# huggingface/transformers

Hardware: AMD Instinct MI355X
Metric: fwd+bwd tokens/sec (whole job), Llama-3-8B seq=4096 (higher is better)
Workload: dtype bf16; 1 GPU; llama3-8b: LlamaForCausalLM fwd+bwd incl. lm_head + causal-LM loss, random-init bf16 weights, per-GPU batch 8 x seq 4096; model=llama3-8b, global_batch=8, seq_len=4096, parallelism=dp1

## Files before the change

transformers_amd/csrc/attention.hip:

```cpp
#include "attention_common.h"

namespace tamd {

#include "attention_fwd_kernel.inc"

}

#include "attention_bwd.inc"

using namespace tamd;

namespace {

#ifdef TAMD_DIAG
unsigned long long* g_attn_trace = nullptr;
#endif

template <typename T, int D>
int attn_fwd_launch(const AttnArgs& a, bool causal, hipStream_t s) {
  const size_t smem = (size_t)4 * kKB * D * 2;
  dim3 grid((unsigned)(a.nqt * a.heads_q * a.batch)), block(kAttnThreads);
  const bool mask = a.key_valid != nullptr;
  const bool drop = a.drop_thr != 0;
#define TAMD_AF(C_, M_, D_) hipLaunchKernelGGL((attn_fwd_kernel<T, D, C_, M_, D_>), grid, block, smem, s, a)
  if (drop) {
    if (causal)
      TAMD_AF(true, true, true);
    else
      TAMD_AF(false, true, true);
  } else if (causal) {
    if (mask)
      TAMD_AF(true, true, false);
    else
      TAMD_AF(true, false, false);
  } else {
    if (mask)
      TAMD_AF(false, true, false);
    else
      TAMD_AF(false, false, false);
  }
#undef TAMD_AF
  return launch_status();
}

template <typename T, int D>
int attn_decode_launch(const AttnArgs& a, bool causal, hipStream_t s) {
  const size_t smem = (size_t)4 * kKB * D * 2;
  dim3 grid((unsigned)(a.nqt * a.heads_q * a.batch * a.kv_splits)), block(kAttnThreads);
#define TAMD_AD(C_, L_) hipLaunchKernelGGL((attn_fwd_kernel<T, D, C_, true, false, true, L_>), grid, block, smem, s, a)
  if (a.seq_k_dev != nullptr) {
    if (causal)
      TAMD_AD(true, true);
    else
      TAMD_AD(false, true);
  } else {
    if (causal)
      TAMD_AD(true, false);
    else
      TAMD_AD(false, false);
  }
#undef TAMD_AD
  const int rows = a.batch * a.seq_q * a.heads_q;
  hipLaunchKernelGGL((attn_combine_kernel<T, D>), dim3((unsigned)rows), dim3(256), 0, s, a);
  return launch_status();
}

int attn_check(const tamd_attn_params* p) {
  if (!p || !p->q || !p->k || !p->v || !p->o) return TAMD_E_NULL;
  if (p->head_dim != 64 && p->head_dim != 128) return TAMD_E_SHAPE;
  if (p->batch <= 0 || p->heads_q <= 0 || p->heads_kv <= 0 || p->seq_q <= 0 || p->seq_k <= 0) return TAMD_E_SHAPE;
  if (p->heads_q % p->heads_kv != 0) return TAMD_E_SHAPE;
  if (p->dtype != TAMD_BF16 && p->dtype != TAMD_F16) return TAMD_E_DTYPE;
  if (!(p->dropout_p >= 0.f && p->dropout_p < 1.f)) return TAMD_E_ARG;
  if (p->q_start != nullptr && (!p->causal || p->seq_q != p->seq_k)) return TAMD_E_ARG;
  const int64_t strides[] = {p->q_stride_b, p->q_stride_s, p->q_stride_h, p->k_stride_b, p->k_stride_s, p->k_stride_h,
                             p->v_stride_b, p->v_stride_s, p->v_stride_h, p->o_stride_b, p->o_stride_s, p->o_stride_h};
  for (int64_t st : strides)
    if (st % 8 != 0) return TAMD_E_ALIGN;
  const int64_t row_strides[] = {p->q_stride_s, p->k_stride_s, p->v_stride_s, p->o_stride_s};
  const int64_t row_counts[] = {p->seq_q, p->seq_k, p->seq_k, p->seq_q};
  for (int i = 0; i < 4; ++i)
    if (row_counts[i] > 1 && (row_strides[i] < p->head_dim || row_strides[i] > ((int64_t)1 << 24))) return TAMD_E_ARG;
  if (!aligned16(p->q) || !aligned16(p->k) || !aligned16(p->v) || !aligned16(p->o)) return TAMD_E_ALIGN;
  return TAMD_OK;
}

AttnArgs make_args(const tamd_attn_params* p) {
  AttnArgs a;
  a.q = p->q;
  a.k = p->k;
  a.v = p->v;
  a.o = p->o;
// ... 159 lines not shown
```

transformers_amd/csrc/attention_bwd.inc:

```

namespace tamd {

#include "attention_bwd_dq_kernel.inc"

template <typename T, int D>
static int attn_bwd_launch(const AttnArgs& a, const tamd_attn_bwd_params* p, bool causal, hipStream_t s) {
  AttnBwdArgs g;
  g.f = a;
  g.dout = p->dout;
  g.dq = p->dq;
  g.dk = p->dk;
  g.dv = p->dv;
  g.delta = p->delta;
  g.scale = p->fwd.scale;
  g.rope_cos = p->rope_cos;
  g.rope_sin = p->rope_sin;
  g.rope_cos_batch = (int)p->rope_cos_batch;
  const bool mask = a.key_valid != nullptr;
  const bool drop = a.drop_thr != 0;
  {
    const size_t smem = (size_t)4 * kKB * D * 2;
    dim3 grid((unsigned)(a.nqt * a.heads_q * a.batch)), block(kAttnThreads);
#define TAMD_DQ(C_, M_, D_) hipLaunchKernelGGL((attn_bwd_dq_kernel<T, D, C_, M_, D_>), grid, block, smem, s, g)
    if (drop) {
      if (causal)
        TAMD_DQ(true, true, true);
      else
        TAMD_DQ(false, true, true);
    } else if (causal) {
      if (mask)
        TAMD_DQ(true, true, false);
      else
        TAMD_DQ(true, false, false);
    } else {
      if (mask)
        TAMD_DQ(false, true, false);
      else
        TAMD_DQ(false, false, false);
    }
#undef TAMD_DQ
  }
  const int st = launch_status();
  return st != 0 ? st : attn_bwd_dkdv_launch(g, __is_same(T, bf16_t) ? TAMD_BF16 : TAMD_F16, D, causal, s);
}

}
```

transformers_amd/csrc/attention_bwd_dq_kernel.inc:

```
template <typename T, int D, bool CAUSAL, bool HAS_MASK, bool DROP>
__global__ __launch_bounds__(kAttnThreads, 2) void attn_bwd_dq_kernel(AttnBwdArgs g) {
  const AttnArgs& a = g.f;
  constexpr int ROWB = D * 2, TILEB = kKB * ROWB, KS = D / 16, DT = D / 32, OROWB = ROWB + 16;
  TAMD_DYN_SMEM(smem);
  const int tid = threadIdx.x, lane = tid & 63;
  const int wave = wave_id_uniform();
  const int hi = lane >> 5, l31 = lane & 31;
  const int group = a.heads_q / a.heads_kv;
  int b, h, qt;
  {
    const int bid = blockIdx.x;
    const int per_grp = a.nqt * group;
    int gi, within;
    if (a.xcd_map) {
      const int xcd = bid & 7, j = bid >> 3;
      gi = (j / per_grp) * 8 + xcd;
      within = j % per_grp;
    } else {
      gi = bid / per_grp;
      within = bid % per_grp;
    }
    b = gi / a.heads_kv;
    h = (gi % a.heads_kv) * group + within % group;
    qt = a.nqt - 1 - within / group;
  }
  const int hkv = h / group;
  const int q0 = qt * kQB, qw0 = q0 + wave * 32, qrow = qw0 + l31;
  const int off = a.seq_k - a.seq_q;
  const T* Q = reinterpret_cast<const T*>(a.q) + (int64_t)b * a.qsb + (int64_t)h * a.qsh;
  const T* K = reinterpret_cast<const T*>(a.k) + (int64_t)b * a.ksb + (int64_t)hkv * a.ksh;
  const T* V = reinterpret_cast<const T*>(a.v) + (int64_t)b * a.vsb + (int64_t)hkv * a.vsh;
  const T* dO = reinterpret_cast<const T*>(g.dout) + (int64_t)b * a.osb + (int64_t)h * a.osh;

  const T* O = reinterpret_cast<const T*>(a.o) + (int64_t)b * a.osb + (int64_t)h * a.osh;
  u32x4 qf[KS], dof[KS];
  float dlt = 0.f;
#pragma unroll
  for (int ks = 0; ks < KS; ++ks) {
    const bool ok = qrow < a.seq_q;
    qf[ks] = ok ? ld16(Q + (int64_t)qrow * a.qss + ks * 16 + hi * 8) : u32x4{0, 0, 0, 0};
    dof[ks] = ok ? ld16(dO + (int64_t)qrow * a.oss + ks * 16 + hi * 8) : u32x4{0, 0, 0, 0};
    const u32x4 of = ok ? ld16(O + (int64_t)qrow * a.oss + ks * 16 + hi * 8) : u32x4{0, 0, 0, 0};
    float x[8], y[8];
    unpack16<T>(of, x);
    unpack16<T>(dof[ks], y);
#pragma unroll
    for (int e = 0; e < 8; ++e) dlt += x[e] * y[e];
  }
  dlt += swap32_f32(dlt);
#pragma unroll
  for (int ks = 0; ks < KS; ++ks) qf[ks] = scale_frag<T>(qf[ks], a.scale_log2, !a.q_prescaled);
  const int64_t stat_idx = ((int64_t)b * a.heads_q + h) * a.seq_q + qrow;
  const float nlse2 = (qrow < a.seq_q) ? -a.lse[stat_idx] * 1.44269504088896340736f : -INFINITY;
  constexpr bool S_FROM_LSE = !(HAS_MASK && D > 64);
  const f32x16 s_start = splat16(S_FROM_LSE ? nlse2 : 0.f);
  constexpr bool FOLD_DELTA = !DROP && !(HAS_MASK && D > 64);
  const f32x16 dp_start = splat16(FOLD_DELTA ? -dlt : 0.f);
  if (hi == 0 && qrow < a.seq_q) {
    g.delta[stat_idx] = -dlt;
    g.delta[(int64_t)a.batch * a.heads_q * a.seq_q + stat_idx] = nlse2;
  }
  const AttnDrop drop = attn_drop_ctx(a);
  const unsigned long long drop_base = drop.row_base((unsigned long long)b * a.heads_q + h, (qrow >> 1) <= ((a.seq_q - 1) >> 1) ? qrow : 0);
  const unsigned drop_lsh = (qrow & 1) ? 0u : 16u;

  const int klo = packed_klo(a, b, qrow);
  const int klo_max = (int)wave_max((float)klo), klo_min = -(int)wave_max(-(float)klo);

  TileOffsets<D> toff;
  toff.init(lane);
  const unsigned lds0 = lds_base_u32(smem);
  f32x16 dqacc[DT];
#pragma unroll
  for (int dt = 0; dt < DT; ++dt)
#pragma unroll
    for (int r = 0; r < 16; ++r) dqacc[dt][r] = 0.f;

  int kend = a.seq_k;
  if (CAUSAL) {
    const int lim = q0 + kQB + off;
    kend = lim < kend ? lim : kend;
    if (kend < 0) kend = 0;
  }
  const int nkt = (kend + kKB - 1) / kKB;
  TileFeed<D> feed, feedv;
  feed.init(a.kss, wave, lane);
  feedv.init(a.vss, wave, lane);
  static_assert(KS == 2 * TileFeed<D>::NI, "one piece per k-step of the first sub-tile");
  auto issue_piece = [&](int t, int rows, int buf, int n) {
    constexpr int NI = TileFeed<D>::NI;
    const unsigned k_off = (unsigned)buf * 2u * TILEB, v_off = k_off + TILEB;
    if (n < NI)
      feed.issue_one_rng(K + (int64_t)t * kKB * a.kss, rows, a.kss, smem, k_off, wave, n);
    else
      feedv.issue_one_rng(V + (int64_t)t * kKB * a.vss, rows, a.vss, smem, v_off, wave, n - NI);
  };
  auto tile_rows = [&](int t) { return a.seq_k - t * kKB < kKB ? a.seq_k - t * kKB : kKB; };
  auto issue = [&](int t, int rows, int buf) {
#pragma unroll
    for (int n = 0; n < KS; ++n) issue_piece(t, rows, buf, n);
  };
  const int t0 = (q0 < a.seq_q ? packed_klo(a, b, q0) : 0) / kKB;
  if (nkt > t0) issue(t0, tile_rows(t0), t0 & 1);
  wait_vmcnt0();
  block_sync();
  for (int t = t0; t < nkt; ++t) {
    const int cur = t & 1;
    const int tn = t + 1, rows_n = t + 1 < nkt ? tile_rows(t + 1) : 0;
    const unsigned k_off = (unsigned)cur * 2u * TILEB, v_off = k_off + TILEB;
    const int kt0 = t * kKB;
    const bool wave_active = (!CAUSAL || (kt0 <= qw0 + 31 + off)) && (kt0 + kKB > klo_min);
    if (!wave_active) issue(tn, rows_n, cur ^ 1);
    if (wave_active) {
      unsigned long long vmask = ~0ull;
      if (HAS_MASK) {
        const int kp = kt0 + lane;
        vmask = ballot64(kp < a.seq_k && (a.key_valid == nullptr || a.key_valid[(int64_t)b * a.seq_k + kp] != 0));
      }
      const bool need_mask = (HAS_MASK && vmask != ~0ull) || (kt0 + kKB > a.seq_k) || (CAUSAL && (kt0 + kKB - 1 > qw0 + off)) ||
                             (kt0 < klo_max);
      const unsigned kb = lds0 + k_off;
      u32x4 dsf[4];
      constexpr int NV = DT * 4;
      constexpr int VA = (DROP || (HAS_MASK && D > 64)) ? 2 : (NV < 4 ? NV : 4);
      u32x4 vr[VA + 1];
      auto creq = [&](int i) -> u32x4 {
        const int dt = i % DT, j = i / DT;
        const int rb = ((j >> 1) * 32 + (j & 1) * 16) * ROWB;
        const u32x2 lo = lds_read8_tr16_abs(kb + toff.tr[dt][0], rb);
        const u32x2 h2 = lds_read8_tr16_abs(kb + toff.tr[dt][1], rb);
        return u32x4{lo[0], lo[1], h2[0], h2[1]};
      };
      {
        constexpr int NA = 4 * KS;
        constexpr int KA = (DROP || (HAS_MASK && D > 64)) ? 2 : 3;
        u32x4 fr[KA + 1];
        auto areq = [&](int i) -> u32x4 {
          const int sub = i / (2 * KS), ks = (i >> 1) % KS;
          return lds_read16_abs(kb + toff.row[ks], sub * 32 * ROWB + (i & 1) * TILEB);
        };
#pragma unroll
        for (int i = 0; i < KA; ++i) fr[i] = areq(i);
#pragma unroll
        for (int sub = 0; sub < 2; ++sub) {
          f32x16 s, dp;
          if (S_FROM_LSE) {
            s = s_start;
          } else {
#pragma unroll
            for (int r = 0; r < 16; ++r) s[r] = 0.f;
          }
          if (FOLD_DELTA) {
            dp = dp_start;
          } else {
#pragma unroll
            for (int r = 0; r < 16; ++r) dp[r] = 0.f;
          }
#pragma unroll
          for (int k2 = 0; k2 < 2 * KS; ++k2) {
            const int i = sub * 2 * KS + k2;
            if (i + KA < NA) fr[(i + KA) % (KA + 1)] = areq(i + KA);
            if (KA >= 3) {
              if (!(i & 1)) constexpr_wait_frag2<KA - 1>(NA - 2 - i, fr[i % (KA + 1)], fr[(i + 1) % (KA + 1)]);
            } else {
              constexpr_wait_frag<KA>(NA - 1 - i, fr[i % (KA + 1)]);
            }
            if (k2 & 1)
              dp = mfma32<T>(fr[i % (KA + 1)], dof[k2 >> 1], dp);
            else
              s = mfma32<T>(fr[i % (KA + 1)], qf[k2 >> 1], s);
            if (sub == 0 && (k2 & 1)) issue_piece(tn, rows_n, cur ^ 1, k2 >> 1);
          }
          if (need_mask) {
#pragma unroll
            for (int r = 0; r < 16; ++r) {
              const int kl = sub * 32 + (r & 3) + 8 * (r >> 2) + 4 * hi;
              const int kp = kt0 + kl;
              bool vis = kp < a.seq_k && kp >= klo;
              if (CAUSAL) vis = vis && (kp <= qrow + off);
              if (HAS_MASK) vis = vis && ((vmask >> kl) & 1ull);
              s[r] = vis ? s[r] : -INFINITY;
            }
          }
          float ds[16];
          if (DROP) {
#pragma unroll
            for (int r = 0; r < 16; r += 4) {
              unsigned w0, w1;
              drop.words(drop_base + (unsigned long long)(((kt0 + sub * 32 + (r & 3) + 8 * (r >> 2) + 4 * hi) >> 1) + (qrow & 1)), w0, w1);
              dp[r] = drop.kept(pair_even_u32(w0), drop_lsh) ? dp[r] : 0.f;
              dp[r + 1] = drop.kept(pair_even_u32(w1), drop_lsh) ? dp[r + 1] : 0.f;
              dp[r + 2] = drop.kept(pair_odd_u32(w0), drop_lsh) ? dp[r + 2] : 0.f;
              dp[r + 3] = drop.kept(pair_odd_u32(w1), drop_lsh) ? dp[r + 3] : 0.f;
            }
          }
#pragma unroll
          for (int r = 0; r < 16; ++r)
            ds[r] = fast_exp2(S_FROM_LSE ? s[r] : s[r] + nlse2) * (DROP ? fmaf(dp[r], drop.scale, -dlt) : (FOLD_DELTA ? dp[r] : dp[r] - dlt));
          pack_c_to_b<T>(ds, &dsf[sub * 2]);
          pin_frags(dsf[sub * 2], dsf[sub * 2 + 1]);
            }
      }
      {
#pragma unroll
        for (int i = 0; i < VA; ++i) vr[i] = creq(i);
#pragma unroll
        for (int i = 0; i < NV; ++i) {
          if (i + VA < NV) vr[(i + VA) % (VA + 1)] = creq(i + VA);
          if (VA >= 3) {
            if (!(i & 1)) constexpr_wait_frag2<2 * (VA - 1)>(2 * (NV - 2 - i), vr[i % (VA + 1)], vr[(i + 1) % (VA + 1)]);
          } else {
            constexpr_wait_frag<2 * VA>(2 * (NV - 1 - i), vr[i % (VA + 1)]);
          }
          dqacc[i % DT] = mfma32<T>(vr[i % (VA + 1)], dsf[i / DT], dqacc[i % DT]);
        }
      }
    }
    wait_vmcnt0();
    block_sync();
  }
  T* dQ = reinterpret_cast<T*>(g.dq) + (int64_t)b * a.qsb + (int64_t)h * a.qsh;
  const int64_t crow0 = (g.rope_cos_batch == 1 ? 0 : (int64_t)b * a.seq_q) + qw0;
  store_rows_via_lds<T, D>(dqacc, g.scale, smem, (unsigned)wave * (32u * OROWB), dQ, a.qss, qw0, a.seq_q, lane,
                           reinterpret_cast<const T*>(g.rope_cos), reinterpret_cast<const T*>(g.rope_sin), crow0);
}
```

transformers_amd/csrc/attention_common.h:

```cpp
#pragma once
#include <stdlib.h>

#include "common.h"
#include "dropout.h"

namespace tamd {

template <int N>
struct IntC {
  static constexpr int value = N;
};

constexpr int kAttnThreads = 256;
constexpr int kQB = 128;
constexpr int kKB = 64;

__device__ __attribute__((aligned(16))) static const unsigned int g_zero16a[4] = {0u, 0u, 0u, 0u};

struct AttnArgs {
  const void* q;
  const void* k;
  const void* v;
  void* o;
  float* lse;
  const uint8_t* key_valid;
  const int* q_start;
  int batch, heads_q, heads_kv, seq_q, seq_k;
  int64_t qsb, qss, qsh, ksb, kss, ksh, vsb, vss, vsh, osb, oss, osh;
  float scale_log2;
  unsigned drop_thr;
  float drop_scale;
  unsigned seed_lo, seed_hi;
  const unsigned long long* seed_dev;
  int nqt;
  int xcd_map;
  int q_prescaled;
  unsigned long long* trace;
  float* o_part;
  float* lse_part;
  int kv_splits, tiles_per_split;
  const int* seq_k_dev;
};

#ifdef TAMD_DIAG
#define TAMD_ATTN_PHASE(i_)                              \
  if (tr) {                                              \
    asm volatile("" ::: "memory");                       \
    const unsigned long long now_ = device_clock();      \
    asm volatile("" ::: "memory");                       \
    ph[i_] += now_ - tlast;                              \
    tlast = now_;                                        \
  }
#else
#define TAMD_ATTN_PHASE(i_)
#endif

__device__ __forceinline__ AttnDrop attn_drop_ctx(const AttnArgs& a) {
  unsigned s0 = a.seed_lo, s1 = a.seed_hi;
  if (a.seed_dev != nullptr) {
    const unsigned long long mixed = attn_seed_mix(*a.seed_dev);
    s0 = (unsigned)mixed;
    s1 = (unsigned)(mixed >> 32);
  }
  return AttnDrop{a.drop_thr << 16, s0, s1, a.drop_scale, ((unsigned long long)a.seq_q + 1) >> 1,
                  ((unsigned long long)a.seq_k + 1) >> 1};
}

template <int D>
__device__ __forceinline__ int row_swz(int row) {
  return D == 128 ? (((row & 3) << 2) | ((row >> 2) & 3)) : ((((row >> 1) & 1) << 2) | ((row >> 2) & 3));
}

template <typename T, int D>
__device__ __forceinline__ void issue_kv_tile(const T* __restrict__ base, int64_t stride, int key0, int nkeys,
                                              char* smem, unsigned tile_off, int wave, int lane) {
  constexpr int ROWB = D * 2;
  constexpr int SLOTS = ROWB / 16;
  constexpr int RPI = 1024 / ROWB;
  constexpr int NI = (kKB * ROWB) / 1024 / 4;
#pragma unroll
  for (int i = 0; i < NI; ++i) {
    const int inst = wave * NI + i;
    const int r = inst * RPI + lane / SLOTS;
    const int p = lane % SLOTS;
    const int s = p ^ row_swz<D>(r);
    const int key = key0 + r;
    const void* src = (key < nkeys) ? (const void*)(base + (int64_t)key * stride + s * 8) : (const void*)g_zero16a;
    glds16(src, smem, tile_off + (unsigned)inst * 1024u);
  }
}

template <int D>
struct TileFeed {
  static constexpr int NI = (kKB * D * 2) / 1024 / 4;
  unsigned voff[NI];
  __device__ __forceinline__ void init(int64_t stride, int wave, int lane) {
    constexpr int ROWB = D * 2, SLOTS = ROWB / 16, RPI = 1024 / ROWB;
#pragma unroll
    for (int i = 0; i < NI; ++i) {
      const int inst = wave * NI + i;
      const int r = inst * RPI + lane / SLOTS;
      const int s = (lane % SLOTS) ^ row_swz<D>(r);
      voff[i] = (unsigned)(((int64_t)r * stride + s * 8) * 2);
    }
  }
  static __host__ __device__ __forceinline__ bool usable(int64_t stride) { return stride > 0 && stride * (kKB * 2) < ((int64_t)1 << 31); }
  template <typename T>
  __device__ __forceinline__ void issue_one(const T* __restrict__ first_row, char* smem, unsigned tile_off, int wave,
                                            int i) const {
    glds16_buf<0>(first_row, voff[i], smem, tile_off + (unsigned)(wave * NI + i) * 1024u);
  }
  template <typename T>
  __device__ __forceinline__ void issue_one_rng(const T* __restrict__ first_row, int rows, int64_t stride, char* smem,
                                                unsigned tile_off, int wave, int i) const {
    glds16_buf_rng(first_row, (unsigned)rows * (unsigned)stride * 2u, voff[i], smem, tile_off + (unsigned)(wave * NI + i) * 1024u);
  }
  template <typename T>
  __device__ __forceinline__ void issue(const T* __restrict__ first_row, char* smem, unsigned tile_off, int wave) const {
#pragma unroll
    for (int i = 0; i < NI; ++i) issue_one(first_row, smem, tile_off, wave, i);
  }
};

template <int D>
struct TileOffsets {
  unsigned row[D / 16];
  unsigned tr[D / 32][2];
  __device__ __forceinline__ void init(int lane) {
    constexpr int ROWB = D * 2;
    const int hi = lane >> 5, l31 = lane & 31, kq = (lane & 15) >> 2;
#pragma unroll
    for (int ks = 0; ks < D / 16; ++ks)
      row[ks] = (unsigned)l31 * ROWB + (unsigned)(((ks * 2 + hi) ^ row_swz<D>(l31)) * 16);
#pragma unroll
    for (int dt = 0; dt < D / 32; ++dt) {
      const int col = dt * 32 + 16 * ((lane >> 4) & 1) + 4 * (lane & 3);
#pragma unroll
      for (int t2 = 0; t2 < 2; ++t2) {
        const int r = 4 * hi + kq + 8 * t2;
        tr[dt][t2] = (unsigned)r * ROWB + (unsigned)(((col >> 3) ^ row_swz<D>(r)) * 16) + (unsigned)(col & 7) * 2u;
      }
    }
  }
  __device__ __forceinline__ u32x4 read_tr(const char* smem, unsigned tile_off, int dt, int j) const {
    const unsigned rb = (unsigned)(((j >> 1) * 32 + (j & 1) * 16) * (D * 2));
    const u32x2 lo = lds_read8_tr16(smem, tile_off + tr[dt][0] + rb);
    const u32x2 h2 = lds_read8_tr16(smem, tile_off + tr[dt][1] + rb);
    return u32x4{lo[0], lo[1], h2[0], h2[1]};
  }
  __device__ __forceinline__ u32x4 read_row(const char* smem, unsigned tile_off, int sub, int ks) const {
    return lds_read16(smem, tile_off + row[ks] + (unsigned)(sub * 32 * D * 2));
  }
};

template <int N>
__device__ __forceinline__ void wait_frag(u32x4& f) {
#if defined(__HIP_DEVICE_COMPILE__)
  asm volatile("s_waitcnt lgkmcnt(%1)" : "+v"(f) : "n"(N) : "memory");
#else
  (void)f;
#endif
}
__device__ __forceinline__ void pin_frags(u32x4& f0, u32x4& f1) {
#if defined(__HIP_DEVICE_COMPILE__)
  asm volatile("" : "+v"(f0), "+v"(f1));
#else
  (void)f0;
  (void)f1;
// ... 142 lines not shown
```

transformers_amd/csrc/attention_fwd_kernel.inc:

```
template <typename T, int D, bool CAUSAL, bool HAS_MASK, bool DROP, bool SPLIT = false, bool DEVLEN = false>
__global__ __launch_bounds__(kAttnThreads, (DROP && D > 64) ? 1 : ((D == 64 && !HAS_MASK && !DROP) ? 3 : 2)) void attn_fwd_kernel(AttnArgs a) {
  constexpr int ROWB = D * 2;
  constexpr int TILEB = kKB * ROWB;
  constexpr int KS = D / 16;
  constexpr int DT = D / 32;
  constexpr int OROWB = ROWB + 16;
  TAMD_DYN_SMEM(smem);
  const int tid = threadIdx.x, lane = tid & 63;
  const int wave = wave_id_uniform();
  const int hi = lane >> 5, l31 = lane & 31;

  const int group = a.heads_q / a.heads_kv;
  int b, h, qt;
  const int split = SPLIT ? (int)(blockIdx.x % (unsigned)a.kv_splits) : 0;
  {
    const int bid = SPLIT ? (int)(blockIdx.x / (unsigned)a.kv_splits) : (int)blockIdx.x;
    const int per_grp = a.nqt * group;
    int g, within;
    if (a.xcd_map) {
      const int xcd = bid & 7, j = bid >> 3;
      g = (j / per_grp) * 8 + xcd;
      within = j % per_grp;
    } else {
      g = bid / per_grp;
      within = bid % per_grp;
    }
    b = g / a.heads_kv;
    const int hkv = g % a.heads_kv;
    h = hkv * group + within % group;
    qt = a.nqt - 1 - within / group;
  }
  const int hkv = h / group;
  const int q0 = qt * kQB;
  static_assert(!DEVLEN || SPLIT, "key counts in device memory: the split-KV instantiations only");
  int seq_k = a.seq_k;
  if constexpr (SPLIT && DEVLEN) {
    int n = wave_uniform_i32(a.seq_k_dev[b]);
    n = n < a.seq_k ? n : a.seq_k;
    seq_k = n > 0 ? n : 0;
  }
  const int off = seq_k - a.seq_q;
  const T* Q = reinterpret_cast<const T*>(a.q) + (int64_t)b * a.qsb + (int64_t)h * a.qsh;
  const T* K = reinterpret_cast<const T*>(a.k) + (int64_t)b * a.ksb + (int64_t)hkv * a.ksh;
  const T* V = reinterpret_cast<const T*>(a.v) + (int64_t)b * a.vsb + (int64_t)hkv * a.vsh;

  const int qw0 = q0 + wave * 32;
  const int qrow = qw0 + l31;
  u32x4 qf[KS];
#pragma unroll
  for (int ks = 0; ks < KS; ++ks)
    qf[ks] = (qrow < a.seq_q) ? ld16(Q + (int64_t)qrow * a.qss + ks * 16 + hi * 8) : u32x4{0, 0, 0, 0};
#pragma unroll
  for (int ks = 0; ks < KS; ++ks) qf[ks] = scale_frag<T>(qf[ks], a.scale_log2, !a.q_prescaled);

  const int klo = packed_klo(a, b, qrow);
  const int klo_max = (int)wave_max((float)klo), klo_min = -(int)wave_max(-(float)klo);

  f32x16 oacc[DT];
#pragma unroll
  for (int dt = 0; dt < DT; ++dt)
#pragma unroll
    for (int r = 0; r < 16; ++r) oacc[dt][r] = 0.f;
  float m_run = -INFINITY, l_run = 0.f;
  f32x16 neg_m = splat16(0.f);

  int kend = seq_k;
  if (CAUSAL) {
    const int lim = q0 + kQB - 1 + off + 1;
    kend = lim < kend ? lim : kend;
    if (kend < 0) kend = 0;
  }
  const int nkt = (kend + kKB - 1) / kKB;

  TileOffsets<D> toff;
  toff.init(lane);
  const unsigned lds0 = lds_base_u32(smem);
  const AttnDrop drop = attn_drop_ctx(a);
  const unsigned long long drop_base = drop.row_base((unsigned long long)b * a.heads_q + h, (qrow >> 1) <= ((a.seq_q - 1) >> 1) ? qrow : 0);
  const unsigned drop_lsh = (qrow & 1) ? 0u : 16u;
  constexpr float kDeferThr = 6.f;

  TileFeed<D> feed, feedv;
  feed.init(a.kss, wave, lane);
  feedv.init(a.vss, wave, lane);
  auto issue_piece = [&](int t, int rows, int buf, int n) {
    constexpr int NI = TileFeed<D>::NI;
    const unsigned k_off = (unsigned)buf * 2u * TILEB, v_off = k_off + TILEB;
    if (n < NI)
      feed.issue_one_rng(K + (int64_t)t * kKB * a.kss, rows, a.kss, smem, k_off, wave, n);
    else
      feedv.issue_one_rng(V + (int64_t)t * kKB * a.vss, rows, a.vss, smem, v_off, wave, n - NI);
  };
  auto tile_rows = [&](int t) { return seq_k - t * kKB < kKB ? seq_k - t * kKB : kKB; };
  auto issue = [&](int t, int rows, int buf) {
#pragma unroll
    for (int n = 0; n < 2 * TileFeed<D>::NI; ++n) issue_piece(t, rows, buf, n);
  };
  const int t0f = (q0 < a.seq_q ? packed_klo(a, b, q0) : 0) / kKB;
  const int t0 = SPLIT ? (t0f > split * a.tiles_per_split ? t0f : split * a.tiles_per_split) : t0f;
  const int nkt_w = SPLIT ? (nkt < (split + 1) * a.tiles_per_split ? nkt : (split + 1) * a.tiles_per_split) : nkt;
  if (nkt_w > t0) issue(t0, tile_rows(t0), t0 & 1);
  wait_vmcnt0();
  block_sync();

#ifdef TAMD_DIAG
  const bool tr = a.trace != nullptr && blockIdx.x == 0;
  unsigned long long ph[8] = {0, 0, 0, 0, 0, 0, 0, 0}, tlast = tr ? device_clock() : 0ull;
#endif
  for (int t = t0; t < nkt_w; ++t) {
    const int cur = t & 1;
    const int tn = t + 1, rows_n = t + 1 < nkt_w ? tile_rows(t + 1) : 0;
    TAMD_ATTN_PHASE(0)
    const unsigned k_off = (unsigned)cur * 2u * TILEB, v_off = k_off + TILEB;
    const int kt0 = t * kKB;
    const bool wave_active = (!CAUSAL || (kt0 <= qw0 + 31 + off)) && (kt0 + kKB > klo_min);
    if (wave_active) {
      const unsigned kb = lds0 + k_off, vb = lds0 + v_off;
      f32x16 s[2] = {neg_m, neg_m};
      {
        constexpr int NM = 2 * KS;
        constexpr int KA = (DROP || (HAS_MASK && D > 64)) ? 2 : (NM < 8 ? NM : 8);
        u32x4 kr[KA + 1];
#pragma unroll
        for (int i = 0; i < KA; ++i) kr[i] = lds_read16_abs(kb + toff.row[i >> 1], (i & 1) * 32 * ROWB);
#pragma unroll
        for (int i = 0; i < NM; ++i) {
          if (i + KA < NM) kr[(i + KA) % (KA + 1)] = lds_read16_abs(kb + toff.row[(i + KA) >> 1], ((i + KA) & 1) * 32 * ROWB);
          if (KA >= 3) {
            if (!(i & 1)) constexpr_wait_frag2<KA - 1>(NM - 2 - i, kr[i % (KA + 1)], kr[(i + 1) % (KA + 1)]);
          } else {
            constexpr_wait_frag<KA>(NM - 1 - i, kr[i % (KA + 1)]);
          }
          s[i & 1] = mfma32<T>(kr[i % (KA + 1)], qf[i >> 1], s[i & 1]);
          if ((i & 1) && (i >> 1) < 2 * TileFeed<D>::NI) issue_piece(tn, rows_n, cur ^ 1, i >> 1);
        }
      }
      TAMD_ATTN_PHASE(1)
      constexpr int NV = DT * 4;
      constexpr int VA = (DROP || (HAS_MASK && D > 64)) ? 2 : (NV < 7 ? NV : 7);
      u32x4 vr[VA + 1];
      auto vreq = [&](int i) -> u32x4 {
        const int dt = i % DT, j = i / DT;
        const int rb = ((j >> 1) * 32 + (j & 1) * 16) * ROWB;
        const u32x2 lo = lds_read8_tr16_abs(vb + toff.tr[dt][0], rb);
        const u32x2 h2 = lds_read8_tr16_abs(vb + toff.tr[dt][1], rb);
        return u32x4{lo[0], lo[1], h2[0], h2[1]};
      };
#pragma unroll
      for (int i = 0; i < VA; ++i) vr[i] = vreq(i);
      unsigned long long vmask = ~0ull;
      if (HAS_MASK) {
        const int kp = kt0 + lane;
        vmask = ballot64(kp < seq_k && (a.key_valid == nullptr || a.key_valid[(int64_t)b * a.seq_k + kp] != 0));
      }
      const bool need_mask = (HAS_MASK && vmask != ~0ull) || (kt0 + kKB > seq_k) || (CAUSAL && (kt0 + kKB - 1 > qw0 + off)) ||
                             (kt0 < klo_max);
      if (need_mask) {
#pragma unroll
        for (int sub = 0; sub < 2; ++sub)
#pragma unroll
          for (int r = 0; r < 16; ++r) {
            const int kl = sub * 32 + (r & 3) + 8 * (r >> 2) + 4 * hi;
            const int kp = kt0 + kl;
            bool vis = kp < seq_k && kp >= klo;
            if (CAUSAL) vis = vis && (kp <= qrow + off);
            if (HAS_MASK) vis = vis && ((vmask >> kl) & 1ull);
            s[sub][r] = vis ? s[sub][r] : -INFINITY;
          }
      }
      float mx = s[0][0];
#pragma unroll
      for (int sub = 0; sub < 2; ++sub)
#pragma unroll
        for (int r = 0; r < 16; ++r) mx = fmaxf(mx, s[sub][r]);
      mx = fmaxf(mx, swap32_f32(mx));
      const float m_old = (m_run == -INFINITY) ? 0.f : m_run;
      const float m_tile = mx + m_old;
      if (ballot64(m_tile - m_run > kDeferThr) != 0ull) {
        const float m_new = fmaxf(m_run, m_tile);
        const float alpha = (m_new == -INFINITY) ? 1.f : fast_exp2(m_run - m_new);
        m_run = m_new;
        l_run *= alpha;
#pragma unroll
        for (int dt = 0; dt < DT; ++dt)
#pragma unroll
          for (int r = 0; r < 16; ++r) oacc[dt][r] *= alpha;
        const float m_ref = (m_new == -INFINITY) ? 0.f : m_new;
        const float shift = m_ref - m_old;
#pragma unroll
        for (int sub = 0; sub < 2; ++sub)
#pragma unroll
          for (int r = 0; r < 16; ++r) s[sub][r] -= shift;
        neg_m = splat16(-m_ref);
      }
      float psum = 0.f;
      u32x4 pf[4];
#pragma unroll
      for (int sub = 0; sub < 2; ++sub) {
        float p[16];
#pragma unroll
        for (int r = 0; r < 16; ++r) {
          p[r] = fast_exp2(s[sub][r]);
          psum += p[r];
        }
        if (DROP) {
#pragma unroll
          for (int r = 0; r < 16; r += 4) {
            unsigned w0, w1;
            drop.words(drop_base + (unsigned long long)(((kt0 + sub * 32 + (r & 3) + 8 * (r >> 2) + 4 * hi) >> 1) + (qrow & 1)), w0, w1);
            p[r] = drop.kept(pair_even_u32(w0), drop_lsh) ? p[r] : 0.f;
            p[r + 1] = drop.kept(pair_even_u32(w1), drop_lsh) ? p[r + 1] : 0.f;
            p[r + 2] = drop.kept(pair_odd_u32(w0), drop_lsh) ? p[r + 2] : 0.f;
            p[r + 3] = drop.kept(pair_odd_u32(w1), drop_lsh) ? p[r + 3] : 0.f;
          }
        }
#pragma unroll
        for (int st = 0; st < 2; ++st)
          pf[sub * 2 + st] = u32x4{pack2<T>(p[8 * st + 0], p[8 * st + 1]), pack2<T>(p[8 * st + 2], p[8 * st + 3]),
                                   pack2<T>(p[8 * st + 4], p[8 * st + 5]), pack2<T>(p[8 * st + 6], p[8 * st + 7])};
      }
      l_run += psum;
      TAMD_ATTN_PHASE(2)
#pragma unroll
      for (int i = 0; i < NV; ++i) {
        if (i + VA < NV) vr[(i + VA) % (VA + 1)] = vreq(i + VA);
        if (VA >= 3) {
          if (!(i & 1)) constexpr_wait_frag2<2 * (VA - 1)>(2 * (NV - 2 - i), vr[i % (VA + 1)], vr[(i + 1) % (VA + 1)]);
        } else {
          constexpr_wait_frag<2 * VA>(2 * (NV - 1 - i), vr[i % (VA + 1)]);
        }
        oacc[i % DT] = mfma32<T>(vr[i % (VA + 1)], pf[i / DT], oacc[i % DT]);
      }
      TAMD_ATTN_PHASE(3)
    } else {
      issue(tn, rows_n, cur ^ 1);
    }
    wait_vmcnt0();
    TAMD_ATTN_PHASE(4)
    block_sync();
    TAMD_ATTN_PHASE(5)
  }
#ifdef TAMD_DIAG
  if (tr && lane == 0) {
#pragma unroll
    for (int i = 0; i < 8; ++i) a.trace[wave * 8 + i] = ph[i];
  }
#endif

  l_run += swap32_f32(l_run);
  const float inv_l = (l_run > 0.f) ? (DROP ? drop.scale : 1.f) / l_run : 0.f;
  if (SPLIT) {
    if (qrow < a.seq_q) {
      const int64_t prow = (((int64_t)split * a.batch + b) * a.seq_q + qrow) * a.heads_q + h;
      if (hi == 0)
        a.lse_part[(((int64_t)split * a.batch + b) * a.heads_q + h) * a.seq_q + qrow] =
            (l_run > 0.f) ? (m_run + fast_log2(l_run)) * 0.69314718055994530942f : -INFINITY;
      float* dst = a.o_part + prow * D;
#pragma unroll
      for (int dt = 0; dt < DT; ++dt)
#pragma unroll
        for (int qd = 0; qd < 4; ++qd)
          st16(dst + dt * 32 + 8 * qd + 4 * hi,
               u32x4{f32_as_u32(oacc[dt][qd * 4 + 0] * inv_l), f32_as_u32(oacc[dt][qd * 4 + 1] * inv_l),
                     f32_as_u32(oacc[dt][qd * 4 + 2] * inv_l), f32_as_u32(oacc[dt][qd * 4 + 3] * inv_l)});
    }
    return;
  }
  if (a.lse != nullptr && hi == 0 && qrow < a.seq_q) {
    const float lse = (l_run > 0.f) ? (m_run + fast_log2(l_run)) * 0.69314718055994530942f : INFINITY;
    a.lse[((int64_t)b * a.heads_q + h) * a.seq_q + qrow] = lse;
  }
  const unsigned st_off = (unsigned)wave * (32u * OROWB);
#pragma unroll
  for (int dt = 0; dt < DT; ++dt)
#pragma unroll
    for (int qd = 0; qd < 4; ++qd) {
      const int d0 = dt * 32 + 8 * qd + 4 * hi;
      const u32x2 pk = {pack2<T>(oacc[dt][qd * 4 + 0] * inv_l, oacc[dt][qd * 4 + 1] * inv_l),
                        pack2<T>(oacc[dt][qd * 4 + 2] * inv_l, oacc[dt][qd * 4 + 3] * inv_l)};
      lds_write8(smem, st_off + (unsigned)l31 * OROWB + (unsigned)d0 * 2u, pk);
    }
  wave_lockstep_point();
  T* O = reinterpret_cast<T*>(a.o) + (int64_t)b * a.osb + (int64_t)h * a.osh;
  constexpr int SLOTS = ROWB / 16;
  constexpr int RPI = 64 / SLOTS;
#pragma unroll
  for (int it = 0; it < 32 / RPI; ++it) {
    const int row = it * RPI + lane / SLOTS, slot = lane % SLOTS;
    const int qr = qw0 + row;
    const u32x4 v = lds_read16(smem, st_off + (unsigned)row * OROWB + (unsigned)slot * 16u);
    if (qr < a.seq_q) st16(O + (int64_t)qr * a.oss + slot * 8, v);
  }
}

template <typename T, int D>
__global__ __launch_bounds__(256) void attn_combine_kernel(AttnArgs a) {
  __shared__ float part[4][D];
  __shared__ float wpart[4];
  const int wave = wave_id_uniform(), lane = threadIdx.x & 63;
  const int row = (int)blockIdx.x;
  const int h = row % a.heads_q, qrow = (row / a.heads_q) % a.seq_q, b = row / (a.heads_q * a.seq_q);
  const int64_t lse_stride = (int64_t)a.batch * a.heads_q * a.seq_q;
  const float* lse0 = a.lse_part + ((int64_t)b * a.heads_q + h) * a.seq_q + qrow;
  float mx = -INFINITY;
  for (int s = lane; s < a.kv_splits; s += 64) mx = fmaxf(mx, lse0[(int64_t)s * lse_stride]);
  mx = wave_max(mx);
  constexpr int PER = D / 64;
  float acc[PER], wsum = 0.f;
#pragma unroll
  for (int e = 0; e < PER; ++e) acc[e] = 0.f;
  const int64_t o_stride = (int64_t)a.batch * a.seq_q * a.heads_q * D;
  const float* o0 = a.o_part + (((int64_t)b * a.seq_q + qrow) * a.heads_q + h) * D + lane * PER;
#pragma unroll 4
  for (int s = wave; s < a.kv_splits; s += 4) {
    const float ls = lse0[(int64_t)s * lse_stride];
    const float w = (ls == -INFINITY) ? 0.f : __expf(ls - mx);
    wsum += w;
    const float* src = o0 + (int64_t)s * o_stride;
#pragma unroll
    for (int e = 0; e < PER; ++e) acc[e] += w * src[e];
  }
#pragma unroll
  for (int e = 0; e < PER; ++e) part[wave][lane * PER + e] = acc[e];
  if (lane == 0) wpart[wave] = wsum;
  block_sync();
  if (wave != 0) return;
  wsum = ((wpart[0] + wpart[1]) + wpart[2]) + wpart[3];
  const float inv = wsum > 0.f ? 1.f / wsum : 0.f;
  T* O = reinterpret_cast<T*>(a.o) + (int64_t)b * a.osb + (int64_t)qrow * a.oss + (int64_t)h * a.osh + lane * PER;
  typedef typename elem<T>::raw raw;
#pragma unroll
  for (int e = 0; e < PER; ++e) {
    const int c = lane * PER + e;
    reinterpret_cast<raw*>(O)[e] = elem<T>::from_f32((((part[0][c] + part[1][c]) + part[2][c]) + part[3][c]) * inv);
  }
  if (a.lse != nullptr && lane == 0)
    a.lse[((int64_t)b * a.heads_q + h) * a.seq_q + qrow] = wsum > 0.f ? mx + __logf(wsum) : INFINITY;
}
```

Before: 25640 tokens/s.

## Restructure attention tile loops with compile-time buffers, packed-doc specialization, and split ranges

Adds a PACKED template parameter so the packed-document bounds (packed_klo/wave_max) compile out when documents aren't packed. The key-tile loop is split into skip, active and trailing-skip ranges computed up front, replacing the per-tile wave_active branch. For causal unmasked D=128 it unrolls by two with compile-time buffer indices so LDS offsets fold into immediates. It also precomputes per-lane LDS base addresses and moves the global-to-LDS piece offsets into the instruction immediate field. This targets scalar/VALU address overhead and divergence in the fwd and dq attention kernels, but adds more template instantiations and code size and may raise register pressure.

```diff
diff --git a/transformers_amd/csrc/attention.hip b/transformers_amd/csrc/attention.hip
--- a/transformers_amd/csrc/attention.hip
+++ b/transformers_amd/csrc/attention.hip
@@ -22,22 +22,30 @@
   dim3 grid((unsigned)(a.nqt * a.heads_q * a.batch)), block(kAttnThreads);
   const bool mask = a.key_valid != nullptr;
   const bool drop = a.drop_thr != 0;
-#define TAMD_AF(C_, M_, D_) hipLaunchKernelGGL((attn_fwd_kernel<T, D, C_, M_, D_>), grid, block, smem, s, a)
-  if (drop) {
+  const bool packed = a.q_start != nullptr;
+#define TAMD_AF(C_, M_, D_, P_) hipLaunchKernelGGL((attn_fwd_kernel<T, D, C_, M_, D_, false, false, P_>), grid, block, smem, s, a)
+  if (packed) {
+    if (drop)
+      TAMD_AF(true, true, true, true);
+    else if (mask)
+      TAMD_AF(true, true, false, true);
+    else
+      TAMD_AF(true, false, false, true);
+  } else if (drop) {
     if (causal)
-      TAMD_AF(true, true, true);
-    else
-      TAMD_AF(false, true, true);
+      TAMD_AF(true, true, true, false);
+    else
+      TAMD_AF(false, true, true, false);
   } else if (causal) {
     if (mask)
-      TAMD_AF(true, true, false);
-    else
-      TAMD_AF(true, false, false);
+      TAMD_AF(true, true, false, false);
+    else
+      TAMD_AF(true, false, false, false);
   } else {
     if (mask)
-      TAMD_AF(false, true, false);
-    else
-      TAMD_AF(false, false, false);
+      TAMD_AF(false, true, false, false);
+    else
+      TAMD_AF(false, false, false, false);
   }
 #undef TAMD_AF
   return launch_status();
diff --git a/transformers_amd/csrc/attention_bwd.inc b/transformers_amd/csrc/attention_bwd.inc
--- a/transformers_amd/csrc/attention_bwd.inc
+++ b/transformers_amd/csrc/attention_bwd.inc
@@ -21,22 +21,30 @@
   {
     const size_t smem = (size_t)4 * kKB * D * 2;
     dim3 grid((unsigned)(a.nqt * a.heads_q * a.batch)), block(kAttnThreads);
-#define TAMD_DQ(C_, M_, D_) hipLaunchKernelGGL((attn_bwd_dq_kernel<T, D, C_, M_, D_>), grid, block, smem, s, g)
-    if (drop) {
+    const bool packed = a.q_start != nullptr;
+#define TAMD_DQ(C_, M_, D_, P_) hipLaunchKernelGGL((attn_bwd_dq_kernel<T, D, C_, M_, D_, P_>), grid, block, smem, s, g)
+    if (packed) {
+      if (drop)
+        TAMD_DQ(true, true, true, true);
+      else if (mask)
+        TAMD_DQ(true, true, false, true);
+      else
+        TAMD_DQ(true, false, false, true);
+    } else if (drop) {
       if (causal)
-        TAMD_DQ(true, true, true);
+        TAMD_DQ(true, true, true, false);
       else
-        TAMD_DQ(false, true, true);
+        TAMD_DQ(false, true, true, false);
     } else if (causal) {
       if (mask)
-        TAMD_DQ(true, true, false);
+        TAMD_DQ(true, true, false, false);
       else
-        TAMD_DQ(true, false, false);
+        TAMD_DQ(true, false, false, false);
     } else {
       if (mask)
-        TAMD_DQ(false, true, false);
+        TAMD_DQ(false, true, false, false);
       else
-        TAMD_DQ(false, false, false);
+        TAMD_DQ(false, false, false, false);
     }
 #undef TAMD_DQ
   }
diff --git a/transformers_amd/csrc/attention_bwd_dq_kernel.inc b/transformers_amd/csrc/attention_bwd_dq_kernel.inc
--- a/transformers_amd/csrc/attention_bwd_dq_kernel.inc
+++ b/transformers_amd/csrc/attention_bwd_dq_kernel.inc
@@ -1,4 +1,4 @@
-template <typename T, int D, bool CAUSAL, bool HAS_MASK, bool DROP>
+template <typename T, int D, bool CAUSAL, bool HAS_MASK, bool DROP, bool PACKED>
 __global__ __launch_bounds__(kAttnThreads, 2) void attn_bwd_dq_kernel(AttnBwdArgs g) {
   const AttnArgs& a = g.f;
   constexpr int ROWB = D * 2, TILEB = kKB * ROWB, KS = D / 16, DT = D / 32, OROWB = ROWB + 16;
@@ -64,12 +64,21 @@
   const unsigned long long drop_base = drop.row_base((unsigned long long)b * a.heads_q + h, (qrow >> 1) <= ((a.seq_q - 1) >> 1) ? qrow : 0);
   const unsigned drop_lsh = (qrow & 1) ? 0u : 16u;
 
-  const int klo = packed_klo(a, b, qrow);
-  const int klo_max = (int)wave_max((float)klo), klo_min = -(int)wave_max(-(float)klo);
+  const int klo = PACKED ? packed_klo(a, b, qrow) : 0;
+  const int klo_max = PACKED ? wave_uniform_i32((int)wave_max((float)klo)) : 0;
+  const int klo_min = PACKED ? wave_uniform_i32(-(int)wave_max(-(float)klo)) : 0;
 
   TileOffsets<D> toff;
   toff.init(lane);
   const unsigned lds0 = lds_base_u32(smem);
+  unsigned arow[KS], atr[DT][2];
+#pragma unroll
+  for (int ks = 0; ks < KS; ++ks) arow[ks] = lds0 + toff.row[ks];
+#pragma unroll
+  for (int dt = 0; dt < DT; ++dt) {
+    atr[dt][0] = lds0 + toff.tr[dt][0];
+    atr[dt][1] = lds0 + toff.tr[dt][1];
+  }
   f32x16 dqacc[DT];
 #pragma unroll
   for (int dt = 0; dt < DT; ++dt)
@@ -100,26 +109,39 @@
 #pragma unroll
     for (int n = 0; n < KS; ++n) issue_piece(t, rows, buf, n);
   };
-  const int t0 = (q0 < a.seq_q ? packed_klo(a, b, q0) : 0) / kKB;
-  if (nkt > t0) issue(t0, tile_rows(t0), t0 & 1);
+  const int t0 = PACKED ? wave_uniform_i32((q0 < a.seq_q ? packed_klo(a, b, q0) : 0) / kKB) : 0;
+  if (nkt > t0) issue(t0, tile_rows(t0), 0);
   wait_vmcnt0();
   block_sync();
-  for (int t = t0; t < nkt; ++t) {
-    const int cur = t & 1;
+  const int xdiag = qw0 + 31 + off;
+  int thi = CAUSAL ? (xdiag < 0 ? 0 : xdiag / kKB + 1) : nkt;
+  thi = thi < nkt ? thi : nkt;
+  int tlo = PACKED ? klo_min / kKB : t0;
+  tlo = tlo > t0 ? tlo : t0;
+  tlo = tlo < nkt ? tlo : nkt;
+  thi = thi > tlo ? thi : tlo;
+  auto skip_tile = [&](int t) __attribute__((always_inline)) {
+    issue(t + 1, t + 1 < nkt ? tile_rows(t + 1) : 0, ((t - t0) & 1) ^ 1);
+    wait_vmcnt0();
+    block_sync();
+  };
+  constexpr bool TWO = !PACKED && !HAS_MASK && !DROP;
+  auto tile = [&](auto cur_c, int t) __attribute__((always_inline)) {
+    constexpr bool RT = __is_same(decltype(cur_c), int);
+    const int cur = buf_of(cur_c);
     const int tn = t + 1, rows_n = t + 1 < nkt ? tile_rows(t + 1) : 0;
-    const unsigned k_off = (unsigned)cur * 2u * TILEB, v_off = k_off + TILEB;
     const int kt0 = t * kKB;
-    const bool wave_active = (!CAUSAL || (kt0 <= qw0 + 31 + off)) && (kt0 + kKB > klo_min);
-    if (!wave_active) issue(tn, rows_n, cur ^ 1);
-    if (wave_active) {
+    {
       unsigned long long vmask = ~0ull;
       if (HAS_MASK) {
         const int kp = kt0 + lane;
         vmask = ballot64(kp < a.seq_k && (a.key_valid == nullptr || a.key_valid[(int64_t)b * a.seq_k + kp] != 0));
       }
+      const unsigned long long vmask_l = HAS_MASK ? (hi ? vmask >> 4 : vmask) : ~0ull;
       const bool need_mask = (HAS_MASK && vmask != ~0ull) || (kt0 + kKB > a.seq_k) || (CAUSAL && (kt0 + kKB - 1 > qw0 + off)) ||
                              (kt0 < klo_max);
-      const unsigned kb = lds0 + k_off;
+      const int kb = RT ? 0 : cur * 2 * TILEB;
+      const unsigned kbv = RT ? (unsigned)cur * 2u * TILEB : 0u;
       u32x4 dsf[4];
       constexpr int NV = DT * 4;
       constexpr int VA = (DROP || (HAS_MASK && D > 64)) ? 2 : (NV < 4 ? NV : 4);
@@ -127,8 +149,8 @@
       auto creq = [&](int i) -> u32x4 {
         const int dt = i % DT, j = i / DT;
         const int rb = ((j >> 1) * 32 + (j & 1) * 16) * ROWB;
-        const u32x2 lo = lds_read8_tr16_abs(kb + toff.tr[dt][0], rb);
-        const u32x2 h2 = lds_read8_tr16_abs(kb + toff.tr[dt][1], rb);
+        const u32x2 lo = lds_read8_tr16_abs(atr[dt][0] + kbv, kb + rb);
+        const u32x2 h2 = lds_read8_tr16_abs(atr[dt][1] + kbv, kb + rb);
         return u32x4{lo[0], lo[1], h2[0], h2[1]};
       };
       {
@@ -137,7 +159,7 @@
         u32x4 fr[KA + 1];
         auto areq = [&](int i) -> u32x4 {
           const int sub = i / (2 * KS), ks = (i >> 1) % KS;
-          return lds_read16_abs(kb + toff.row[ks], sub * 32 * ROWB + (i & 1) * TILEB);
+          return lds_read16_abs(arow[ks] + kbv, kb + sub * 32 * ROWB + (i & 1) * TILEB);
         };
 #pragma unroll
         for (int i = 0; i < KA; ++i) fr[i] = areq(i);
@@ -178,7 +200,7 @@
               const int kp = kt0 + kl;
               bool vis = kp < a.seq_k && kp >= klo;
               if (CAUSAL) vis = vis && (kp <= qrow + off);
-              if (HAS_MASK) vis = vis && ((vmask >> kl) & 1ull);
+              if (HAS_MASK) vis = vis && ((vmask_l >> (kl - 4 * hi)) & 1ull);
               s[r] = vis ? s[r] : -INFINITY;
             }
           }
@@ -218,6 +240,23 @@
     }
     wait_vmcnt0();
     block_sync();
+  };
+  {
+    int t = t0;
+    if constexpr (!TWO) {
+      for (; t < tlo; ++t) skip_tile(t);
+      for (; t < thi; ++t) tile((t - t0) & 1, t);
+    } else {
+      for (; t + 1 < thi; t += 2) {
+        tile(IntC<0>{}, t);
+        tile(IntC<1>{}, t + 1);
+      }
+      if (t < thi) {
+        tile(IntC<0>{}, t);
+        ++t;
+      }
+    }
+    for (; t < nkt; ++t) skip_tile(t);
   }
   T* dQ = reinterpret_cast<T*>(g.dq) + (int64_t)b * a.qsb + (int64_t)h * a.qsh;
   const int64_t crow0 = (g.rope_cos_batch == 1 ? 0 : (int64_t)b * a.seq_q) + qw0;
diff --git a/transformers_amd/csrc/attention_common.h b/transformers_amd/csrc/attention_common.h
--- a/transformers_amd/csrc/attention_common.h
+++ b/transformers_amd/csrc/attention_common.h
@@ -10,6 +10,10 @@
 struct IntC {
   static constexpr int value = N;
 };
+
+template <int N>
+__host__ __device__ constexpr int buf_of(IntC<N>) { return N; }
+__host__ __device__ constexpr int buf_of(int n) { return n; }
 
 constexpr int kAttnThreads = 256;
 constexpr int kQB = 128;
@@ -90,9 +94,20 @@
   }
 }
 
+template <int IMM>
+__device__ __forceinline__ void glds16_buf_rng_imm(const void* base, unsigned bytes, unsigned voff, char* smem, unsigned lds_base_off) {
+#if defined(__HIP_DEVICE_COMPILE__)
+  const __amdgpu_buffer_rsrc_t r = __builtin_amdgcn_make_buffer_rsrc(const_cast<void*>(base), (short)0, (int)bytes, 0x00020000);
+  __builtin_amdgcn_raw_ptr_buffer_load_lds(r, (__attribute__((address_space(3))) void*)(smem + lds_base_off), 16, (int)voff, 0, IMM, 0);
+#else
+  glds16_buf_rng(base, bytes, voff + (unsigned)IMM, smem, lds_base_off + (unsigned)IMM);
+#endif
+}
+
 template <int D>
 struct TileFeed {
   static constexpr int NI = (kKB * D * 2) / 1024 / 4;
+  static_assert(NI <= 4, "piece i rides in the 12-bit offset field as i * 1024");
   unsigned voff[NI];
   __device__ __forceinline__ void init(int64_t stride, int wave, int lane) {
     constexpr int ROWB = D * 2, SLOTS = ROWB / 16, RPI = 1024 / ROWB;
@@ -101,19 +116,31 @@
       const int inst = wave * NI + i;
       const int r = inst * RPI + lane / SLOTS;
       const int s = (lane % SLOTS) ^ row_swz<D>(r);
-      voff[i] = (unsigned)(((int64_t)r * stride + s * 8) * 2);
+      voff[i] = (unsigned)(((int64_t)r * stride + s * 8) * 2) - (unsigned)i * 1024u;
     }
   }
   static __host__ __device__ __forceinline__ bool usable(int64_t stride) { return stride > 0 && stride * (kKB * 2) < ((int64_t)1 << 31); }
   template <typename T>
   __device__ __forceinline__ void issue_one(const T* __restrict__ first_row, char* smem, unsigned tile_off, int wave,
                                             int i) const {
-    glds16_buf<0>(first_row, voff[i], smem, tile_off + (unsigned)(wave * NI + i) * 1024u);
+    const unsigned dst = tile_off + (unsigned)(wave * NI) * 1024u;
+    switch (i) {
+      case 0: glds16_buf<0>(first_row, voff[0], smem, dst); break;
+      case 1: glds16_buf<1024>(first_row, voff[1 % NI], smem, dst); break;
+      case 2: glds16_buf<2048>(first_row, voff[2 % NI], smem, dst); break;
+      default: glds16_buf<3072>(first_row, voff[3 % NI], smem, dst); break;
+    }
   }
   template <typename T>
   __device__ __forceinline__ void issue_one_rng(const T* __restrict__ first_row, int rows, int64_t stride, char* smem,
                                                 unsigned tile_off, int wave, int i) const {
-    glds16_buf_rng(first_row, (unsigned)rows * (unsigned)stride * 2u, voff[i], smem, tile_off + (unsigned)(wave * NI + i) * 1024u);
+    const unsigned bytes = (unsigned)rows * (unsigned)stride * 2u, dst = tile_off + (unsigned)(wave * NI) * 1024u;
+    switch (i) {
+      case 0: glds16_buf_rng_imm<0>(first_row, bytes, voff[0], smem, dst); break;
+      case 1: glds16_buf_rng_imm<1024>(first_row, bytes, voff[1 % NI], smem, dst); break;
+      case 2: glds16_buf_rng_imm<2048>(first_row, bytes, voff[2 % NI], smem, dst); break;
+      default: glds16_buf_rng_imm<3072>(first_row, bytes, voff[3 % NI], smem, dst); break;
+    }
   }
   template <typename T>
   __device__ __forceinline__ void issue(const T* __restrict__ first_row, char* smem, unsigned tile_off, int wave) const {
diff --git a/transformers_amd/csrc/attention_fwd_kernel.inc b/transformers_amd/csrc/attention_fwd_kernel.inc
--- a/transformers_amd/csrc/attention_fwd_kernel.inc
+++ b/transformers_amd/csrc/attention_fwd_kernel.inc
@@ -1,4 +1,4 @@
-template <typename T, int D, bool CAUSAL, bool HAS_MASK, bool DROP, bool SPLIT = false, bool DEVLEN = false>
+template <typename T, int D, bool CAUSAL, bool HAS_MASK, bool DROP, bool SPLIT = false, bool DEVLEN = false, bool PACKED = false>
 __global__ __launch_bounds__(kAttnThreads, (DROP && D > 64) ? 1 : ((D == 64 && !HAS_MASK && !DROP) ? 3 : 2)) void attn_fwd_kernel(AttnArgs a) {
   constexpr int ROWB = D * 2;
   constexpr int TILEB = kKB * ROWB;
@@ -53,8 +53,10 @@
 #pragma unroll
   for (int ks = 0; ks < KS; ++ks) qf[ks] = scale_frag<T>(qf[ks], a.scale_log2, !a.q_prescaled);
 
-  const int klo = packed_klo(a, b, qrow);
-  const int klo_max = (int)wave_max((float)klo), klo_min = -(int)wave_max(-(float)klo);
+  static_assert(!PACKED || !SPLIT, "packed documents: not in the split-KV instantiations");
+  const int klo = PACKED ? packed_klo(a, b, qrow) : 0;
+  const int klo_max = PACKED ? wave_uniform_i32((int)wave_max((float)klo)) : 0;
+  const int klo_min = PACKED ? wave_uniform_i32(-(int)wave_max(-(float)klo)) : 0;
 
   f32x16 oacc[DT];
 #pragma unroll
@@ -75,6 +77,14 @@
   TileOffsets<D> toff;
   toff.init(lane);
   const unsigned lds0 = lds_base_u32(smem);
+  unsigned arow[KS], atr[DT][2];
+#pragma unroll
+  for (int ks = 0; ks < KS; ++ks) arow[ks] = lds0 + toff.row[ks];
+#pragma unroll
+  for (int dt = 0; dt < DT; ++dt) {
+    atr[dt][0] = lds0 + toff.tr[dt][0];
+    atr[dt][1] = lds0 + toff.tr[dt][1];
+  }
   const AttnDrop drop = attn_drop_ctx(a);
   const unsigned long long drop_base = drop.row_base((unsigned long long)b * a.heads_q + h, (qrow >> 1) <= ((a.seq_q - 1) >> 1) ? qrow : 0);
   const unsigned drop_lsh = (qrow & 1) ? 0u : 16u;
@@ -96,10 +106,10 @@
 #pragma unroll
     for (int n = 0; n < 2 * TileFeed<D>::NI; ++n) issue_piece(t, rows, buf, n);
   };
-  const int t0f = (q0 < a.seq_q ? packed_klo(a, b, q0) : 0) / kKB;
+  const int t0f = PACKED ? wave_uniform_i32((q0 < a.seq_q ? packed_klo(a, b, q0) : 0) / kKB) : 0;
   const int t0 = SPLIT ? (t0f > split * a.tiles_per_split ? t0f : split * a.tiles_per_split) : t0f;
   const int nkt_w = SPLIT ? (nkt < (split + 1) * a.tiles_per_split ? nkt : (split + 1) * a.tiles_per_split) : nkt;
-  if (nkt_w > t0) issue(t0, tile_rows(t0), t0 & 1);
+  if (nkt_w > t0) issue(t0, tile_rows(t0), 0);
   wait_vmcnt0();
   block_sync();
 
@@ -107,25 +117,41 @@
   const bool tr = a.trace != nullptr && blockIdx.x == 0;
   unsigned long long ph[8] = {0, 0, 0, 0, 0, 0, 0, 0}, tlast = tr ? device_clock() : 0ull;
 #endif
-  for (int t = t0; t < nkt_w; ++t) {
-    const int cur = t & 1;
+  const int xdiag = qw0 + 31 + off;
+  int thi = CAUSAL ? (xdiag < 0 ? 0 : xdiag / kKB + 1) : nkt_w;
+  thi = thi < nkt_w ? thi : nkt_w;
+  int tlo = PACKED ? klo_min / kKB : t0;
+  tlo = tlo > t0 ? tlo : t0;
+  tlo = tlo < nkt_w ? tlo : nkt_w;
+  thi = thi > tlo ? thi : tlo;
+  auto skip_tile = [&](int t) __attribute__((always_inline)) {
+    TAMD_ATTN_PHASE(0)
+    issue(t + 1, t + 1 < nkt_w ? tile_rows(t + 1) : 0, ((t - t0) & 1) ^ 1);
+    wait_vmcnt0();
+    TAMD_ATTN_PHASE(4)
+    block_sync();
+    TAMD_ATTN_PHASE(5)
+  };
+  constexpr bool TWO = !PACKED && !SPLIT && !HAS_MASK && !DROP && CAUSAL && D == 128;
+  auto tile = [&](auto cur_c, int t) __attribute__((always_inline)) {
+    constexpr bool RT = __is_same(decltype(cur_c), int);
+    const int cur = buf_of(cur_c);
     const int tn = t + 1, rows_n = t + 1 < nkt_w ? tile_rows(t + 1) : 0;
     TAMD_ATTN_PHASE(0)
-    const unsigned k_off = (unsigned)cur * 2u * TILEB, v_off = k_off + TILEB;
     const int kt0 = t * kKB;
-    const bool wave_active = (!CAUSAL || (kt0 <= qw0 + 31 + off)) && (kt0 + kKB > klo_min);
-    if (wave_active) {
-      const unsigned kb = lds0 + k_off, vb = lds0 + v_off;
+    {
+      const int kb = RT ? 0 : cur * 2 * TILEB, vb = kb + TILEB;
+      const unsigned kbv = RT ? (unsigned)cur * 2u * TILEB : 0u;
       f32x16 s[2] = {neg_m, neg_m};
       {
         constexpr int NM = 2 * KS;
         constexpr int KA = (DROP || (HAS_MASK && D > 64)) ? 2 : (NM < 8 ? NM : 8);
         u32x4 kr[KA + 1];
 #pragma unroll
-        for (int i = 0; i < KA; ++i) kr[i] = lds_read16_abs(kb + toff.row[i >> 1], (i & 1) * 32 * ROWB);
+        for (int i = 0; i < KA; ++i) kr[i] = lds_read16_abs(arow[i >> 1] + kbv, kb + (i & 1) * 32 * ROWB);
 #pragma unroll
         for (int i = 0; i < NM; ++i) {
-          if (i + KA < NM) kr[(i + KA) % (KA + 1)] = lds_read16_abs(kb + toff.row[(i + KA) >> 1], ((i + KA) & 1) * 32 * ROWB);
+          if (i + KA < NM) kr[(i + KA) % (KA + 1)] = lds_read16_abs(arow[(i + KA) >> 1] + kbv, kb + ((i + KA) & 1) * 32 * ROWB);
           if (KA >= 3) {
             if (!(i & 1)) constexpr_wait_frag2<KA - 1>(NM - 2 - i, kr[i % (KA + 1)], kr[(i + 1) % (KA + 1)]);
           } else {
@@ -142,8 +168,8 @@
       auto vreq = [&](int i) -> u32x4 {
         const int dt = i % DT, j = i / DT;
         const int rb = ((j >> 1) * 32 + (j & 1) * 16) * ROWB;
-        const u32x2 lo = lds_read8_tr16_abs(vb + toff.tr[dt][0], rb);
-        const u32x2 h2 = lds_read8_tr16_abs(vb + toff.tr[dt][1], rb);
+        const u32x2 lo = lds_read8_tr16_abs(atr[dt][0] + kbv, vb + rb);
+        const u32x2 h2 = lds_read8_tr16_abs(atr[dt][1] + kbv, vb + rb);
         return u32x4{lo[0], lo[1], h2[0], h2[1]};
       };
 #pragma unroll
@@ -153,6 +179,7 @@
         const int kp = kt0 + lane;
         vmask = ballot64(kp < seq_k && (a.key_valid == nullptr || a.key_valid[(int64_t)b * a.seq_k + kp] != 0));
       }
+      const unsigned long long vmask_l = HAS_MASK ? (hi ? vmask >> 4 : vmask) : ~0ull;
       const bool need_mask = (HAS_MASK && vmask != ~0ull) || (kt0 + kKB > seq_k) || (CAUSAL && (kt0 + kKB - 1 > qw0 + off)) ||
                              (kt0 < klo_max);
       if (need_mask) {
@@ -164,7 +191,7 @@
             const int kp = kt0 + kl;
             bool vis = kp < seq_k && kp >= klo;
             if (CAUSAL) vis = vis && (kp <= qrow + off);
-            if (HAS_MASK) vis = vis && ((vmask >> kl) & 1ull);
+            if (HAS_MASK) vis = vis && ((vmask_l >> (kl - 4 * hi)) & 1ull);
             s[sub][r] = vis ? s[sub][r] : -INFINITY;
           }
       }
@@ -232,13 +259,28 @@
         oacc[i % DT] = mfma32<T>(vr[i % (VA + 1)], pf[i / DT], oacc[i % DT]);
       }
       TAMD_ATTN_PHASE(3)
-    } else {
-      issue(tn, rows_n, cur ^ 1);
     }
     wait_vmcnt0();
     TAMD_ATTN_PHASE(4)
     block_sync();
     TAMD_ATTN_PHASE(5)
+  };
+  {
+    int t = t0;
+    if constexpr (!TWO) {
+      for (; t < tlo; ++t) skip_tile(t);
+      for (; t < thi; ++t) tile((t - t0) & 1, t);
+    } else {
+      for (; t + 1 < thi; t += 2) {
+        tile(IntC<0>{}, t);
+        tile(IntC<1>{}, t + 1);
+      }
+      if (t < thi) {
+        tile(IntC<0>{}, t);
+        ++t;
+      }
+    }
+    for (; t < nkt_w; ++t) skip_tile(t);
   }
 #ifdef TAMD_DIAG
   if (tr && lane == 0) {
@@ -247,38 +289,39 @@
   }
 #endif
 
+  const int lane_e = lane_id_mbcnt(), hi_e = lane_e >> 5, l31_e = lane_e & 31, qrow_e = qw0 + l31_e;
   l_run += swap32_f32(l_run);
   const float inv_l = (l_run > 0.f) ? (DROP ? drop.scale : 1.f) / l_run : 0.f;
   if (SPLIT) {
-    if (qrow < a.seq_q) {
-      const int64_t prow = (((int64_t)split * a.batch + b) * a.seq_q + qrow) * a.heads_q + h;
-      if (hi == 0)
-        a.lse_part[(((int64_t)split * a.batch + b) * a.heads_q + h) * a.seq_q + qrow] =
+    if (qrow_e < a.seq_q) {
+      const int64_t prow = (((int64_t)split * a.batch + b) * a.seq_q + qrow_e) * a.heads_q + h;
+      if (hi_e == 0)
+        a.lse_part[(((int64_t)split * a.batch + b) * a.heads_q + h) * a.seq_q + qrow_e] =
             (l_run > 0.f) ? (m_run + fast_log2(l_run)) * 0.69314718055994530942f : -INFINITY;
       float* dst = a.o_part + prow * D;
 #pragma unroll
       for (int dt = 0; dt < DT; ++dt)
 #pragma unroll
         for (int qd = 0; qd < 4; ++qd)
-          st16(dst + dt * 32 + 8 * qd + 4 * hi,
+          st16(dst + dt * 32 + 8 * qd + 4 * hi_e,
                u32x4{f32_as_u32(oacc[dt][qd * 4 + 0] * inv_l), f32_as_u32(oacc[dt][qd * 4 + 1] * inv_l),
                      f32_as_u32(oacc[dt][qd * 4 + 2] * inv_l), f32_as_u32(oacc[dt][qd * 4 + 3] * inv_l)});
     }
     return;
   }
-  if (a.lse != nullptr && hi == 0 && qrow < a.seq_q) {
+  if (a.lse != nullptr && hi_e == 0 && qrow_e < a.seq_q) {
     const float lse = (l_run > 0.f) ? (m_run + fast_log2(l_run)) * 0.69314718055994530942f : INFINITY;
-    a.lse[((int64_t)b * a.heads_q + h) * a.seq_q + qrow] = lse;
+    a.lse[((int64_t)b * a.heads_q + h) * a.seq_q + qrow_e] = lse;
   }
   const unsigned st_off = (unsigned)wave * (32u * OROWB);
 #pragma unroll
   for (int dt = 0; dt < DT; ++dt)
 #pragma unroll
     for (int qd = 0; qd < 4; ++qd) {
-      const int d0 = dt * 32 + 8 * qd + 4 * hi;
+      const int d0 = dt * 32 + 8 * qd + 4 * hi_e;
       const u32x2 pk = {pack2<T>(oacc[dt][qd * 4 + 0] * inv_l, oacc[dt][qd * 4 + 1] * inv_l),
                         pack2<T>(oacc[dt][qd * 4 + 2] * inv_l, oacc[dt][qd * 4 + 3] * inv_l)};
-      lds_write8(smem, st_off + (unsigned)l31 * OROWB + (unsigned)d0 * 2u, pk);
+      lds_write8(smem, st_off + (unsigned)l31_e * OROWB + (unsigned)d0 * 2u, pk);
     }
   wave_lockstep_point();
   T* O = reinterpret_cast<T*>(a.o) + (int64_t)b * a.osb + (int64_t)h * a.osh;
@@ -286,7 +329,7 @@
   constexpr int RPI = 64 / SLOTS;
 #pragma unroll
   for (int it = 0; it < 32 / RPI; ++it) {
-    const int row = it * RPI + lane / SLOTS, slot = lane % SLOTS;
+    const int row = it * RPI + lane_e / SLOTS, slot = lane_e % SLOTS;
     const int qr = qw0 + row;
     const u32x4 v = lds_read16(smem, st_off + (unsigned)row * OROWB + (unsigned)slot * 16u);
     if (qr < a.seq_q) st16(O + (int64_t)qr * a.oss + slot * 8, v);
```

After: 25710 tokens/s (median of 6 runs). Within noise of the previous version (+0.3%).
